# roeiherz/CanonicalSg2Im

Measured on AMD Instinct MI355X. Metric: 256x256 images/sec/node (G+D step), higher is better.
Workload: dtype f32; 1 GPU; BASELINE config C3: COCO-shaped AttSPADE 256x256, batch 16/GPU, 1-30 objects/img, ngf=64 ndf=64, --no_vgg_loss --use_img_disc 0; Sg2Layout GCN + SPADE G + 2-scale PatchGAN D + object-crop D, fwd+bwd+Adam; global_batch=16, parallelism=dp1

## Files before the change

canonicalsg2im_amd/_lib.py:

```python
import ctypes
import os

import torch

_HERE = os.path.dirname(os.path.abspath(__file__))
LIB_PATH = os.environ.get("CSG_HIP_LIB") or os.path.join(_HERE, "libcsg_hip.so")

MAX_TAPS = 16
ACT_NONE, ACT_LEAKY, ACT_TANH = 0, 1, 2

c_i32, c_i64, c_f32, c_f64, c_p = ctypes.c_int32, ctypes.c_int64, ctypes.c_float, ctypes.c_double, ctypes.c_void_p


class ConvDesc(ctypes.Structure):
    _fields_ = [
        ("B", c_i32), ("IHp", c_i32), ("IWp", c_i32), ("Cin", c_i32), ("x_cs", c_i32),
        ("IHv", c_i32), ("IWv", c_i32), ("in_up", c_i32),
        ("OHg", c_i32), ("OWg", c_i32), ("OHf", c_i32), ("OWf", c_i32), ("os", c_i32), ("ooy", c_i32), ("oox", c_i32),
        ("Cout", c_i32), ("y_cs", c_i32),
        ("istride", c_i32), ("ntaps", c_i32), ("wtaps", c_i32),
        ("tap_dy", c_i32 * MAX_TAPS), ("tap_dx", c_i32 * MAX_TAPS), ("tap_w", c_i32 * MAX_TAPS),
        ("act", c_i32), ("slope", c_f32), ("accumulate", c_i32), ("res_gate", c_i32),
    ]

# ... 19 lines not shown

class SnFwdItem(ctypes.Structure):
    _fields_ = [("w", c_p), ("u", c_p), ("v", c_p), ("Cout", c_i64), ("K", c_i64), ("w_eff", c_p), ("cl_Cin", c_i64),
                ("sigma", c_p), ("u_used", c_p), ("v_used", c_p), ("workspace", c_p), ("workspace_bytes", c_i64)]


class SnBwdItem(ctypes.Structure):
    _fields_ = [("dweff", c_p), ("Cout", c_i64), ("Cin", c_i64), ("KH", c_i64), ("KW", c_i64), ("s0", c_i64), ("s1", c_i64),
                ("s2", c_i64), ("s3", c_i64), ("w", c_p), ("u_used", c_p), ("v_used", c_p), ("sigma", c_p), ("dw", c_p),
                ("workspace", c_p), ("workspace_bytes", c_i64)]


class GemmDesc(ctypes.Structure):
    _fields_ = [("M", ctypes.c_int64), ("N", ctypes.c_int64), ("K", ctypes.c_int64),
                ("lda", ctypes.c_int64), ("ldb", ctypes.c_int64), ("ldy", ctypes.c_int64), ("ldg", ctypes.c_int64),
                ("act", ctypes.c_int32), ("slope", ctypes.c_float), ("gate_slope", ctypes.c_float)]


SIGNATURES = {
    "csg_version": (c_i32, []),
    "csg_last_error": (ctypes.c_char_p, []),
    "csg_prof_enable": (c_i32, [c_i32]),
    "csg_prof_reset": (c_i32, []),
    "csg_prof_num_kernels": (c_i32, []),
    "csg_prof_kernel_name": (ctypes.c_char_p, [c_i32]),
    "csg_prof_read": (c_i32, [c_i32, ctypes.POINTER(c_f64), ctypes.POINTER(c_i64), ctypes.POINTER(c_f64)]),
    "csg_embed_fwd": (c_i32, [c_p, c_i64, c_i64, c_p, c_i64, c_i64, c_p, c_i64, c_i64, c_p]),
    "csg_embed_bwd_workspace": (c_i64, [c_i64, c_i64, c_i64]),
    "csg_embed_bwd": (c_i32, [c_p, c_i64, c_i64, c_p, c_i64, c_i64, c_i64, c_i64, c_p, c_p, c_i64, c_p]),
    "csg_real_object_mask": (c_i32, [c_p, c_i64, c_i64, c_i64, c_i64, c_p, c_p]),
    "csg_graph_csr_build": (c_i32, [c_p, c_i64, c_i64, c_i64, c_p, c_p, c_p]),
    "csg_gather_concat_fwd": (c_i32, [c_p, c_p, c_p, c_i64, c_i64, c_i64, c_i64, c_i64, c_p, c_p]),
    "csg_gather_concat_bwd_workspace": (c_i64, [c_i64, c_i64, c_i64, c_i64]),
    "csg_gather_concat_bwd": (c_i32, [c_p, c_p, c_p, c_i64, c_i64, c_i64, c_i64, c_i64, c_p, c_p, c_p, c_i64, c_p]),
    "csg_segment_avg_fwd_workspace": (c_i64, [c_i64, c_i64, c_i64, c_i64]),
    "csg_segment_avg_fwd": (c_i32, [c_p, c_p, c_p, c_p, c_p, c_i64, c_i64, c_i64, c_i64, c_i64, c_p, c_p, c_p, c_p,
                                    c_i64, c_p]),
    "csg_segment_avg_bwd": (c_i32, [c_p, c_p, c_p, c_p, c_p, c_p, c_p, c_p, c_i64, c_i64, c_i64, c_i64, c_i64, c_i32,
                                    c_p, c_p, c_p, c_p]),
    "csg_layout_fwd": (c_i32, [c_p, c_p, c_p, c_p, c_i64, c_i64, c_i64, c_i64, c_i64, c_i64, c_i64, c_i64, c_p, c_i64,
                               c_i64, c_p]),
    "csg_disc_input_fwd": (c_i32, [c_p, c_p, c_p, c_p, c_i64, c_i64, c_i64, c_i64, c_i64, c_i64, c_p, c_i64, c_i64, c_i64,
                                   c_i64, c_p, c_i64, c_p]),
    "csg_layout_bwd_workspace": (c_i64, [c_i64, c_i64, c_i64, c_i64, c_i64, c_i32, c_i32]),
    "csg_layout_bwd": (c_i32, [c_p, c_i64, c_i64, c_p, c_p, c_p, c_i64, c_i64, c_i64, c_i64, c_i64, c_i64, c_i64,
                               c_i64, c_p, c_i32, c_p, c_p, c_p, c_i64, c_p]),
    "csg_layout_bwd_masks": (c_i32, [c_p, c_i64, c_i64, c_p, c_p, c_i64, c_i64, c_i64, c_i64, c_i64, c_i64, c_i64, c_i64,
                                     c_p, c_p, c_i32, c_p]),
    "csg_layout_mass": (c_i32, [c_p, c_p, c_p, c_p, c_i64, c_i64, c_i64, c_i64, c_i64, c_i64, c_p, c_p]),
    "csg_layout_paint": (c_i32, [c_p, c_p, c_p, c_i64, c_p, c_i64, c_i64, c_i64, c_i64, c_i64, c_i64, c_i64, c_p, c_i64,
                                 c_i64, c_p]),
    "csg_conv_fwd_workspace": (c_i64, [ctypes.POINTER(ConvDesc)]),
    "csg_conv_fwd": (c_i32, [ctypes.POINTER(ConvDesc), c_p, c_p, c_p, c_p, c_p, c_p, c_i64, c_p]),
    "csg_conv_bwd_weight_workspace": (c_i64, [ctypes.POINTER(ConvDesc)]),
    "csg_conv_bwd_weight": (c_i32, [ctypes.POINTER(ConvDesc), c_p, c_p, c_p, c_p, c_p, c_i64, c_p]),
    "csg_wino_pack_bytes": (c_i64, [c_i64, c_i64]),
    "csg_wino_pack_weights": (c_i32, [c_p, c_i64, c_i64, c_i64, c_i64, c_i64, c_i64, c_i32, c_p, c_p, c_p]),
    "csg_conv_fwd_multi_workspace": (c_i64, [ctypes.POINTER(ConvDesc), c_i32]),
    "csg_conv_fwd_multi": (c_i32, [ctypes.POINTER(ConvDesc), c_i32, c_p, c_p, c_p, c_p, c_p, c_p, c_i64, c_p]),
    "csg_gemm_supported": (c_i32, [ctypes.POINTER(GemmDesc)]),
    "csg_gemm_nt": (c_i32, [ctypes.POINTER(GemmDesc), c_p, c_p, c_p, c_p, c_p, c_p]),
    "csg_gemm_tn_workspace": (c_i64, [c_i64, c_i64, c_i64]),
    "csg_gemm_tn": (c_i32, [c_i64, c_i64, c_i64, c_p, c_i64, c_p, c_i64, c_p, c_p, c_p, c_i64, c_p]),
    "csg_conv_few_supported": (c_i32, [ctypes.POINTER(FewDesc)]),
    "csg_conv_few_fwd_workspace": (c_i64, [ctypes.POINTER(FewDesc)]),
    "csg_conv_few_fwd": (c_i32, [ctypes.POINTER(FewDesc), c_p, c_p, c_p, c_p, c_p, c_i64, c_p]),
    "csg_conv_few_bwd_data": (c_i32, [ctypes.POINTER(FewDesc), c_p, c_p, c_p, c_p]),
    "csg_conv_few_bwd_weight_workspace": (c_i64, [ctypes.POINTER(FewDesc)]),
    "csg_conv_few_bwd_weight": (c_i32, [ctypes.POINTER(FewDesc), c_p, c_p, c_p, c_p, c_p, c_i64, c_p]),
    "csg_wino_conv_workspace": (c_i64, [ctypes.POINTER(WinoDesc)]),
    "csg_wino_conv": (c_i32, [ctypes.POINTER(WinoDesc), c_p, c_p, c_p, c_p, c_p, c_f32, c_p, c_p, c_i64, c_p]),
    "csg_wino_bwd_weight_workspace": (c_i64, [ctypes.POINTER(WinoDesc)]),
    "csg_wino_bwd_weight": (c_i32, [ctypes.POINTER(WinoDesc), c_p, c_p, c_p, c_p, c_p, c_i64, c_p]),
    "csg_wino4_bwd_weight_workspace": (c_i64, [ctypes.POINTER(WinoDesc)]),
    "csg_wino4_bwd_weight": (c_i32, [ctypes.POINTER(WinoDesc), c_p, c_p, c_p, c_p, c_p, c_i64, c_p]),
    "csg_wino4_supported": (c_i32, [ctypes.POINTER(WinoDesc)]),
    "csg_wino4_persistent": (c_i32, [c_i32]),
    "csg_wino_pack_weights_multi": (c_i32, [ctypes.POINTER(WinoPackItem), c_i32, c_p]),
    "csg_wino4_pack_bytes": (c_i64, [c_i64, c_i64]),
    "csg_wino4_pack_weights": (c_i32, [c_p, c_i64, c_i64, c_i64, c_i64, c_i64, c_i64, c_i32, c_p, c_p, c_p]),
    "csg_wino4_conv_workspace": (c_i64, [ctypes.POINTER(WinoDesc)]),
    "csg_wino4_conv": (c_i32, [ctypes.POINTER(WinoDesc), c_p, c_p, c_p, c_p, c_p, c_f32, c_p, c_p, c_i64, c_p]),
    "csg_wino4_conv_part": (c_i32, [ctypes.POINTER(WinoDesc), c_p, c_p, c_i64, c_i64, c_p, c_p, c_p, c_i64, c_p, c_p, c_f32,
                                    c_p, c_p]),
    "csg_wino4_conv_spade_supported": (c_i32, [ctypes.POINTER(WinoDesc)]),
    "csg_wino4_conv_spade": (c_i32, [ctypes.POINTER(WinoDesc), c_p, c_p, c_p, c_p, c_p, c_i64, c_p, c_p, c_f32, c_p, c_p]),
    "csg_wino34_supported": (c_i32, [ctypes.POINTER(WinoDesc), c_i32]),
    "csg_wino34_pack_weights": (c_i32, [c_p, c_i64, c_i64, c_i64, c_i64, c_i64, c_i64, c_i32, c_p, c_p, c_p]),
    "csg_wino34_conv_workspace": (c_i64, [ctypes.POINTER(WinoDesc), c_i32]),
    "csg_wino34_conv": (c_i32, [ctypes.POINTER(WinoDesc), c_i32, c_p, c_p, c_p, c_p, c_p, c_f32, c_p, c_p, c_i64, c_p]),
    "csg_act_bwd": (c_i32, [c_p, c_p, c_i64, c_i32, c_f32, c_p, c_p]),
    "csg_colsum": (c_i32, [c_p, c_i64, c_i64, c_i64, c_p, c_p, c_i64, c_p]),
    "csg_norm_stats": (c_i32, [c_p, c_i64, c_i64, c_i64, c_p, c_p, c_i64, c_p]),
    "csg_norm_finalize": (c_i32, [c_p, c_i64, c_i64, c_f64, c_f32, c_i32, c_p, c_p, c_p, c_p, c_f32, c_p]),
    "csg_norm_stats_finalize": (c_i32, [c_p, c_i64, c_i64, c_i64, c_p, c_i64, c_f64, c_f32, c_p, c_p, c_p, c_p, c_p, c_p, c_f32,
                                        c_p]),
    "csg_norm_apply_fwd": (c_i32, [c_p, c_p, c_p, c_p, c_f32, c_i64, c_i64, c_i64, c_p, c_p, c_f32, c_p, c_p]),
    "csg_norm_apply_bwd_reduce": (c_i32, [c_p, c_p, c_p, c_p, c_p, c_p, c_f32, c_i64, c_i64, c_i64, c_p, c_p, c_p, c_i64,
                                          c_i64, c_p]),
    "csg_norm_apply_bwd_dx": (c_i32, [c_p, c_p, c_p, c_p, c_p, c_f32, c_p, c_f64, c_i64, c_i64, c_i64, c_p, c_p, c_p, c_f32,
                                      c_p, c_p, c_i64, c_p]),
    "csg_nearest_resize_fwd": (c_i32, [c_p, c_i64, c_i64, c_i64, c_i64, c_i64, c_i64, c_p, c_p]),
    "csg_nearest_resize_bwd": (c_i32, [c_p, c_i64, c_i64, c_i64, c_i64, c_i64, c_i64, c_p, c_p]),
    "csg_upsample2x_fwd": (c_i32, [c_p, c_i64, c_i64, c_i64, c_i64, c_p, c_p]),
    "csg_upsample2x_bwd": (c_i32, [c_p, c_i64, c_i64, c_i64, c_i64, c_p, c_p]),
    "csg_avgpool3s2_fwd": (c_i32, [c_p, c_i64, c_i64, c_i64, c_i64, c_p, c_p]),
    "csg_avgpool3s2_bwd": (c_i32, [c_p, c_i64, c_i64, c_i64, c_i64, c_p, c_p]),
    "csg_avgpool3s2_bwd_add": (c_i32, [c_p, c_i64, c_i64, c_i64, c_i64, c_p, c_p, c_p]),
    "csg_crop_fwd": (c_i32, [c_p, c_i64, c_i64, c_i64, c_i64, c_i64, c_p, c_p, c_i64, c_i64, c_i64, c_p, c_i64, c_p]),
    "csg_crop_bwd": (c_i32, [c_p, c_i64, c_i64, c_i64, c_i64, c_i64, c_p, c_p, c_i64, c_i64, c_i64, c_i64, c_p, c_p]),
    "csg_crop_bwd_boxes": (c_i32, [c_p, c_p, c_i64, c_i64, c_i64, c_i64, c_i64, c_p, c_p, c_i64, c_i64, c_i64, c_i64, c_p,
                                   c_p]),
    "csg_maxpool2_fwd": (c_i32, [c_p, c_i64, c_i64, c_i64, c_i64, c_p, c_p]),
    "csg_maxpool2_bwd": (c_i32, [c_p, c_p, c_i64, c_i64, c_i64, c_i64, c_p, c_p]),
    "csg_avgpool2_fwd": (c_i32, [c_p, c_i64, c_i64, c_i64, c_i64, c_p, c_p]),
    "csg_avgpool2_bwd": (c_i32, [c_p, c_i64, c_i64, c_i64, c_i64, c_p, c_p]),
    "csg_l1_mean_workspace": (c_i64, [c_i64]),
    "csg_l1_mean_fwd": (c_i32, [c_p, c_p, c_i64, c_p, c_p, c_i64, c_p]),
    "csg_l1_mean_bwd": (c_i32, [c_p, c_p, c_p, c_i64, c_p, c_p]),
    "csg_hinge_mean_fwd": (c_i32, [ctypes.POINTER(HingeItem), c_i32, c_i32, c_p, c_p]),
    "csg_hinge_mean_bwd": (c_i32, [ctypes.POINTER(HingeItem), c_i32, c_i32, c_p, c_p]),
    "csg_spectral_norm_workspace": (c_i64, [c_i64, c_i64]),
    "csg_spectral_norm_fwd": (c_i32, [c_p, c_p, c_p, c_i64, c_i64, c_i32, c_f32, c_p, c_i64, c_p, c_p, c_p, c_p, c_i64,
                                      c_p]),
    "csg_spectral_norm_bwd": (c_i32, [c_p, c_i64, c_i64, c_i64, c_i64, c_i64, c_i64, c_i64, c_i64, c_p, c_p, c_p, c_p,
                                      c_p, c_p, c_i64, c_p]),
    "csg_spectral_norm_fwd_multi": (c_i32, [ctypes.POINTER(SnFwdItem), c_i32, c_i32, c_f32, c_p]),
    "csg_spectral_norm_bwd_multi": (c_i32, [ctypes.POINTER(SnBwdItem), c_i32, c_p]),
    "csg_canon_workspace": (c_i64, [c_i64]),
    "csg_canon_build": (c_i32, [c_p, c_p, c_p, c_p, c_i64, c_i64, ctypes.POINTER(c_i32), c_i64, c_i32, c_i32, c_p, c_i64,
                                c_p, c_p]),
    "csg_canon_emit": (c_i32, [c_p, c_p, c_i64, c_i64, ctypes.POINTER(c_i32), c_i64, c_i32, c_i32, c_p, c_p, c_i64, c_p,
                               c_p, c_p]),
    "csg_canon_converse": (c_i32, [c_p, c_p, c_i64, c_i64, ctypes.POINTER(c_i32), c_i64, c_i32, c_i32, c_p, c_p, c_p, c_p,
                                   c_i64, c_p, c_p, c_p]),
    "csg_canon_general_workspace": (c_i64, [c_i64, c_i64, c_i64]),
    "csg_canon_general_build": (c_i32, [c_p, c_p, c_p, c_p, c_i64, c_i64, c_p, c_p, c_i64, ctypes.POINTER(c_i32), c_i64,
                                        c_i64, c_i32, c_p, c_i64, c_p, c_p]),
    "csg_canon_general_converse": (c_i32, [c_i64, ctypes.POINTER(c_i32), c_i64, c_p, c_i64, c_p, c_p, c_p, c_p, c_p]),
    "csg_canon_general_close": (c_i32, [c_i64, ctypes.POINTER(c_i32), c_i64, c_i32, c_p, c_i64, c_p, c_p]),
    "csg_canon_general_emit": (c_i32, [c_i64, ctypes.POINTER(c_i32), c_i64, c_p, c_i64, c_p, c_i64, c_p, c_p, c_p]),
}


def _load():
    if not os.path.exists(LIB_PATH):
        raise ImportError(
            "libcsg_hip.so is not built (%s). Run `python -c 'import __graft_entry__ as g; g.build()'` "
            "from the repository root; there is no CPU fallback." % LIB_PATH)
    lib = ctypes.CDLL(LIB_PATH)
    for name, (res, args) in SIGNATURES.items():
        fn = getattr(lib, name)
        fn.restype = res
        fn.argtypes = args
    return lib


lib = _load()


def last_error():
    return lib.csg_last_error().decode("utf-8", "replace")


def check(rc, what=""):
    if rc != 0:
        raise RuntimeError("libcsg_hip %s failed (%d): %s" % (what, rc, last_error()))


def ptr(t):
    if t is None:
        return None
    if not t.is_cuda:
        raise RuntimeError("canonicalsg2im_amd ops need HIP (cuda) tensors; got a %s tensor — there is no CPU path"
                           % t.device)
    return ctypes.c_void_p(t.data_ptr())


_raw_stream = getattr(torch._C, "_cuda_getCurrentRawStream", None)


def stream():
    if _raw_stream is not None:
        return ctypes.c_void_p(_raw_stream(torch.cuda.current_device()))
    return ctypes.c_void_p(torch.cuda.current_stream().cuda_stream)


def prof_enable(on=True):
    check(lib.csg_prof_enable(int(on)), "prof_enable")


def prof_reset():
    check(lib.csg_prof_reset(), "prof_reset")


def prof_read():
    out = {}
    for k in range(lib.csg_prof_num_kernels()):
        ms, n, w = c_f64(), c_i64(), c_f64()
        check(lib.csg_prof_read(k, ctypes.byref(ms), ctypes.byref(n), ctypes.byref(w)), "prof_read")
        if n.value:
            out[lib.csg_prof_kernel_name(k).decode()] = (ms.value, n.value, w.value)
    return out
```

canonicalsg2im_amd/csrc/igemm.hip:

```cpp
#include <stddef.h>
#include <stdlib.h>

#include <type_traits>

#include "csg_common.h"
#include "csg_reduce.h"

using namespace csg;

typedef __attribute__((ext_vector_type(16))) float f32x16;
typedef float f32x4 __attribute__((ext_vector_type(4)));
typedef int i32x4 __attribute__((ext_vector_type(4)));

__device__ f32x4 csg_buffer_load_f32x4(i32x4 rsrc, int voffset, int soffset, int aux) __asm(
    "llvm.amdgcn.raw.buffer.load.v4f32");

__device__ __forceinline__ i32x4 make_srd(const void* base, unsigned bytes) {
  const unsigned long long a = (unsigned long long)base;
  i32x4 r;
  r.x = (int)(a & 0xffffffffu);
  r.y = (int)((a >> 32) & 0xffffu);
  r.z = (int)bytes;
  r.w = 0x00020000;
  return r;
}

#define IG_BM 128
#define IG_BK 32
#define IG_LD 36
#define OOB_OFF 0x80000000u
#define MAX_RECORDS 0x7FFFFFF0ll

struct FastDiv {
  unsigned m, s1, s2;
};
static FastDiv make_fastdiv(unsigned d) {
  FastDiv f;
  unsigned l = 0;
  while ((1ull << l) < d) ++l;
  f.m = (unsigned)(((1ull << 32) * ((1ull << l) - d)) / d + 1);
  f.s1 = l < 1 ? l : 1;
  f.s2 = l > 0 ? l - 1 : 0;
  return f;
}
__device__ __forceinline__ unsigned fdiv(unsigned n, const FastDiv& f) {
  unsigned t = __umulhi(f.m, n);
  return (t + ((n - t) >> f.s1)) >> f.s2;
}

struct IgemmParams {
  csg_conv_desc d;
  int M, Ktot, wrow;
  int mtiles, ntiles;
  int simple_out;
  int ksplit, kt_per_split;
// ... 557 lines not shown
  }
  const int left = ch1 - ch;
  if (left == 3) {
    load_tile(ch + 2, ra0, rb0);
    compute_store(buf, ra1, rb1);
    __syncthreads();
    compute_store(buf ^ 1, ra0, rb0);
    __syncthreads();
    compute_tile(buf);
  } else if (left == 2) {
    compute_store(buf, ra1, rb1);
    __syncthreads();
    compute_tile(buf ^ 1);
  } else if (left == 1) {
    compute_tile(buf);
  }

  float* slab = out + (long long)sp * d.Cout * p.wrow;
#pragma unroll
  for (int mi = 0; mi < MI; ++mi) {
    const int n = it * BI + wi * (MI * 32) + r * MI + mi;
    if (n >= d.Cout) continue;
    float* srow = slab + (long long)n * p.wrow;
#pragma unroll
    for (int g = 0; g < 4; ++g)
#pragma unroll
      for (int f = 0; f < NJ; ++f) {
        const int kk = jt * 128 + wj * (NJ * 32) + (8 * g + 4 * hh) * NJ + 4 * f;
        if (kk < p.Ktot) {
          const int sl = kk / d.Cin;
          const int col = s_tap[32 + sl] * d.Cin + (kk - sl * d.Cin);
          float v[4];
#pragma unroll
          for (int e = 0; e < 4; ++e) {
            const int L = 4 * f + e;
            v[e] = acc[mi][L % NJ][4 * g + L / NJ];
          }
          *(float4*)(srow + col) = make_float4(v[0], v[1], v[2], v[3]);
        }
      }
  }
  if (do_db) {
    __syncthreads();
    f32x4* red = (f32x4*)smem;
    red[apr * CQ + ac4] = csum;
    __syncthreads();
    if (apr == 0 && n0 < d.Cout) {
      f32x4 tot = red[ac4];
      for (int q = 1; q < RP; ++q) tot += red[q * CQ + ac4];
      *(f32x4*)(dbp + (long long)sp * d.Cout + n0) = tot;
    }
  }
}

static int validate(const csg_conv_desc* d, const char* who) {
  CSG_REQUIRE(d != nullptr, CSG_E_BADSHAPE, "%s: null descriptor", who);
  CSG_REQUIRE(d->B > 0 && d->IHp > 0 && d->IWp > 0 && d->Cin > 0 && d->Cout > 0 && d->OHg > 0 && d->OWg > 0,
              CSG_E_BADSHAPE, "%s: non-positive dimension", who);
  CSG_REQUIRE(d->Cin % 4 == 0 && d->x_cs % 4 == 0 && d->x_cs >= d->Cin, CSG_E_UNSUPPORTED,
              "%s: Cin=%d and x_cs=%d must be multiples of 4 (16-byte channel rows)", who, d->Cin, d->x_cs);
  CSG_REQUIRE(d->ntaps >= 1 && d->ntaps <= CSG_MAX_TAPS && d->wtaps >= 1, CSG_E_UNSUPPORTED, "%s: ntaps=%d", who,
              d->ntaps);
  CSG_REQUIRE(d->in_up >= 0 && d->in_up <= 4 && d->os >= 1 && d->istride >= 1, CSG_E_BADSHAPE, "%s: bad strides", who);
  CSG_REQUIRE(d->y_cs >= d->Cout, CSG_E_BADSHAPE, "%s: y_cs < Cout", who);
  for (int t = 0; t < d->ntaps; ++t)
    CSG_REQUIRE(d->tap_w[t] >= 0 && d->tap_w[t] < d->wtaps, CSG_E_BADSHAPE, "%s: tap_w out of range", who);
  int64_t M = (int64_t)d->B * d->OHg * d->OWg;
  CSG_REQUIRE(M < (1ll << 31) - 256, CSG_E_UNSUPPORTED, "%s: too many output pixels", who);
  CSG_REQUIRE((int64_t)d->B * d->OHf * d->OWf < (1ll << 31), CSG_E_UNSUPPORTED, "%s: output too large", who);
  const int64_t img_bytes = (int64_t)d->IHp * d->IWp * d->x_cs * 4;
  const int64_t npix = (int64_t)d->OHg * d->OWg;
  const int64_t span = (127 / npix + 2) * img_bytes;
  CSG_REQUIRE(span < MAX_RECORDS, CSG_E_UNSUPPORTED, "%s: one input image is too large for 32-bit offsets", who);
  CSG_REQUIRE((int64_t)d->Cout * d->wtaps * d->Cin * 4 < MAX_RECORDS, CSG_E_UNSUPPORTED, "%s: weights too large", who);
  return CSG_OK;
}

static void fill(IgemmParams& p, const csg_conv_desc* d) {
  p.d = *d;
  p.M = d->B * d->OHg * d->OWg;
  p.Ktot = d->ntaps * d->Cin;
  p.wrow = d->wtaps * d->Cin;
  p.simple_out = (d->os == 1 && d->ooy == 0 && d->oox == 0 && d->OHg == d->OHf && d->OWg == d->OWf) ? 1 : 0;
  p.ksplit = 1;
  p.kt_per_split = (p.Ktot + IG_BK - 1) / IG_BK;
  p.div_ow = make_fastdiv((unsigned)d->OWg);
  p.div_oh = make_fastdiv((unsigned)d->OHg);
  p.img_bytes = (unsigned)((int64_t)d->IHp * d->IWp * d->x_cs * 4);
  p.mtiles = p.ntiles = 0;
  p.ws_off = 0;
  p.tail_tile0 = p.tail_ks = p.tail_kt_per = p.tail_m0 = 0;
}

static int pick_bn(int cout) { return cout <= 32 ? 32 : (cout <= 64 ? 64 : 128); }

static int pick_split(int blocks, int steps, int min_steps, int max_split) {
  int best = 1;
  double best_cost = 1e30;
  for (int s = 1; s <= max_split && steps / s >= min_steps; ++s) {
    const double rounds = (double)((blocks * (long long)s + 511) / 512);
    const double cost = rounds * ((steps + s - 1) / s) + 0.25 * s;
    if (cost < best_cost * 0.97) {
      best_cost = cost;
      best = s;
    }
  }
// ... 78 lines not shown
}

static int pick_bi(int cout) { return cout <= 32 ? 32 : (cout <= 64 ? 64 : 128); }

static int multi_plan(const csg_conv_desc* descs, int n, IgemmMulti& mp, int64_t& ws_floats, int& max_blocks,
                      const char* who) {
  CSG_REQUIRE(descs != nullptr && n >= 1 && n <= IG_MAXCLS, CSG_E_BADSHAPE, "%s: 1..%d descriptors", who, IG_MAXCLS);
  int64_t blocks_total = 0;
  for (int c = 0; c < n; ++c) {
    int rc = validate(&descs[c], who);
    if (rc) return rc;
    CSG_REQUIRE(descs[c].Cout == descs[0].Cout && descs[c].Cin == descs[0].Cin && descs[c].x_cs == descs[0].x_cs &&
                    descs[c].y_cs == descs[0].y_cs && descs[c].wtaps == descs[0].wtaps && descs[c].B == descs[0].B,
                CSG_E_BADSHAPE, "%s: the descriptors must share channels, strides, weights and batch", who);
    fill(mp.p[c], &descs[c]);
    const int bn = pick_bn(descs[c].Cout);
    mp.p[c].mtiles = (mp.p[c].M + IG_BM - 1) / IG_BM;
    mp.p[c].ntiles = (descs[c].Cout + bn - 1) / bn;
    blocks_total += (int64_t)mp.p[c].mtiles * mp.p[c].ntiles;
  }
  for (int c = n; c < IG_MAXCLS; ++c) mp.p[c] = mp.p[0];
  ws_floats = 0;
  max_blocks = 0;
  for (int c = 0; c < n; ++c) {
    IgemmParams& p = mp.p[c];
    const int nkt = (p.Ktot + IG_BK - 1) / IG_BK;
    int ks = 1;
    if (blocks_total < 1024 && nkt >= 16 && p.d.Cout % 4 == 0) ks = pick_split((int)blocks_total, nkt, 8, 64);
    p.kt_per_split = (nkt + ks - 1) / ks;
    p.ksplit = (nkt + p.kt_per_split - 1) / p.kt_per_split;
    p.ws_off = ws_floats;
    if (p.ksplit > 1) ws_floats += (int64_t)p.ksplit * p.M * p.d.Cout;
    const int blocks = p.mtiles * p.ntiles * p.ksplit;
    if (blocks > max_blocks) max_blocks = blocks;
  }
  return CSG_OK;
}

template <int BN>
static int launch_fwd_multi(IgemmMulti& mp, int n, int max_blocks, const float* x, const float* w, const float* bias,
                            const float* res, float* y, float* ws, hipStream_t s) {
  static bool attr_set = false;
  size_t shm = (size_t)(2 * IG_BM * IG_LD + 2 * BN * IG_LD) * 4 + 48 * 4;
  if (!attr_set) {
    hipError_t e = hipFuncSetAttribute((const void*)k_igemm_fwd<BN, true>, hipFuncAttributeMaxDynamicSharedMemorySize, (int)shm);
    CSG_REQUIRE(e == hipSuccess, CSG_E_LAUNCH, "csg_conv_fwd_multi: hipFuncSetAttribute(%zu bytes of LDS): %s", shm, hipGetErrorString(e));
    attr_set = true;
  }
  CSG_LAUNCH((k_igemm_fwd<BN, true>), dim3((unsigned)max_blocks, (unsigned)n), dim3(256), shm, s, mp, x, w, bias, res,
                     y, ws);
  return check_launch("csg_conv_fwd_multi");
}

extern "C" {

int64_t csg_conv_fwd_workspace(const csg_conv_desc* d) {
  if (validate(d, "csg_conv_fwd_workspace")) return -1;
  IgemmParams p;
  fill(p, d);
  fwd_plan(p);
  return fwd_slab_floats(p) * 4;
}

int csg_conv_fwd(const csg_conv_desc* d, const float* x, const float* w, const float* bias, const float* residual,
                 float* y, float* workspace, int64_t workspace_bytes, void* stream) {
  int rc = validate(d, "csg_conv_fwd");
  if (rc) return rc;
  CSG_REQUIRE(((uintptr_t)x % 16) == 0 && ((uintptr_t)w % 16) == 0, CSG_E_UNSUPPORTED,
              "csg_conv_fwd: x and w must be 16-byte aligned");
  CSG_REQUIRE(!d->res_gate || (d->act == CSG_ACT_NONE && residual != nullptr && !d->accumulate), CSG_E_UNSUPPORTED,
              "csg_conv_fwd: res_gate needs act == NONE, a residual (the gating tensor) and no accumulation");
  IgemmParams p;
  fill(p, d);
  fwd_plan(p);
  const int64_t need = fwd_slab_floats(p) * 4;
  CSG_REQUIRE(need == 0 || (workspace != nullptr && workspace_bytes >= need), CSG_E_WORKSPACE,
              "csg_conv_fwd: needs %lld bytes of workspace (csg_conv_fwd_workspace), got %lld", (long long)need,
              (long long)workspace_bytes);
  hipStream_t s = (hipStream_t)stream;
  const int bn = pick_bn(d->Cout);
  {
    ProfScope ps(bn == 128 ? K_IGEMM_FWD : K_IGEMM_FWD64, 2.0 * p.M * (double)p.Ktot * d->Cout, s);
    if (bn == 32)
      rc = launch_fwd<32>(p, x, w, bias, residual, y, workspace, s);
    else if (bn == 64)
      rc = launch_fwd<64>(p, x, w, bias, residual, y, workspace, s);
    else
      rc = launch_fwd<128>(p, x, w, bias, residual, y, workspace, s);
    if (rc) return rc;
  }
  if (p.ksplit > 1 || p.tail_ks > 1) {
    ProfScope ps(K_SPLITK_EPI, (double)fwd_slab_floats(p) * 4 + (double)(p.M - p.tail_m0) * d->Cout * 4, s);
    const int64_t n4 = (int64_t)(p.M - p.tail_m0) * d->Cout / 4;
    int64_t g = cdiv(n4, 256);
    if (g > 4096) g = 4096;
    CSG_LAUNCH(k_splitk_epilogue<false>, dim3((unsigned)g), dim3(256), 0, s, p, workspace, bias, residual, y);
    rc = check_launch("csg_conv_fwd(split-K epilogue)");
  }
  return rc;
}

int64_t csg_conv_fwd_multi_workspace(const csg_conv_desc* descs, int32_t n) {
  IgemmMulti mp;
  int64_t wsf = 0;
  int mb = 0;
  if (multi_plan(descs, n, mp, wsf, mb, "csg_conv_fwd_multi_workspace")) return -1;
  return wsf * 4;
}

int csg_conv_fwd_multi(const csg_conv_desc* descs, int32_t n, const float* x, const float* w, const float* bias,
                       const float* residual, float* y, float* workspace, int64_t workspace_bytes, void* stream) {
  IgemmMulti mp;
  int64_t wsf = 0;
  int mb = 0;
  int rc = multi_plan(descs, n, mp, wsf, mb, "csg_conv_fwd_multi");
  if (rc) return rc;
  CSG_REQUIRE(((uintptr_t)x % 16) == 0 && ((uintptr_t)w % 16) == 0, CSG_E_UNSUPPORTED,
              "csg_conv_fwd_multi: x and w must be 16-byte aligned");
  CSG_REQUIRE(wsf == 0 || (workspace != nullptr && workspace_bytes >= wsf * 4), CSG_E_WORKSPACE,
              "csg_conv_fwd_multi: needs %lld bytes of workspace", (long long)(wsf * 4));
  hipStream_t s = (hipStream_t)stream;
  const int bn = pick_bn(descs[0].Cout);
  double flops = 0.0;
  bool any_split = false;
  int64_t max_n4 = 0;
  for (int c = 0; c < n; ++c) {
    flops += 2.0 * mp.p[c].M * (double)mp.p[c].Ktot * descs[c].Cout;
    any_split = any_split || mp.p[c].ksplit > 1;
    const int64_t n4 = (int64_t)mp.p[c].M * descs[c].Cout / 4;
    if (n4 > max_n4) max_n4 = n4;
  }
  {
    ProfScope ps(bn == 128 ? K_IGEMM_FWD : K_IGEMM_FWD64, flops, s);
// ... 80 lines not shown
```

include/csg_hip.h:

```cpp
#ifndef CSG_HIP_H
#define CSG_HIP_H

#include <stdint.h>

#ifdef __cplusplus
extern "C" {
#endif

#define CSG_OK 0
#define CSG_E_BADSHAPE (-1)
#define CSG_E_UNSUPPORTED (-2)
#define CSG_E_LAUNCH (-3)
#define CSG_E_WORKSPACE (-4)

#define CSG_ACT_NONE 0
#define CSG_ACT_LEAKY 1
#define CSG_ACT_TANH 2

#define CSG_MAX_TAPS 16

int csg_version(void);
const char* csg_last_error(void);

int csg_prof_enable(int mode);
// ... 18 lines not shown
int csg_gather_concat_fwd(const float* obj, const float* pred, const int64_t* triplets, int64_t B, int64_t O,
                          int64_t T, int64_t Din, int64_t Dp, float* out, void* stream);
int64_t csg_gather_concat_bwd_workspace(int64_t B, int64_t O, int64_t T, int64_t Din);
int csg_gather_concat_bwd(const float* dcat, const int32_t* row_ptr, const int32_t* col, int64_t B, int64_t O,
                          int64_t T, int64_t Din, int64_t Dp, float* dobj, float* dpred, void* workspace,
                          int64_t workspace_bytes, void* stream);

int64_t csg_segment_avg_fwd_workspace(int64_t B, int64_t O, int64_t T, int64_t H);
int csg_segment_avg_fwd(const float* h, const float* conf, const uint8_t* valid, const int32_t* row_ptr,
                        const int32_t* col, int64_t B, int64_t O, int64_t T, int64_t H, int64_t Dp, float* pooled,
                        float* cnt, float* new_p, void* workspace, int64_t workspace_bytes, void* stream);
int csg_segment_avg_bwd(const float* dpooled, const float* dnew_p, const float* h, const float* conf,
                        const uint8_t* valid, const int64_t* triplets, const float* pooled, const float* cnt,
                        int64_t B, int64_t O, int64_t T, int64_t H, int64_t Dp, int32_t gate_relu, float* dh,
                        float* dconf, float* dcnt_scratch, void* stream);

int csg_layout_fwd(const float* vecs, const float* boxes, const uint8_t* valid, const float* masks, int64_t M,
                   int64_t B, int64_t O, int64_t S, int64_t H, int64_t W, int64_t OH, int64_t OW, float* out,
                   int64_t out_cs, int64_t out_off, void* stream);
int csg_disc_input_fwd(const float* vecs, const float* boxes, const uint8_t* valid, const float* masks, int64_t M, int64_t B,
                       int64_t O, int64_t S, int64_t H, int64_t W, const float* img, int64_t img_sb, int64_t img_sc,
                       int64_t img_sh, int64_t img_sw, float* out, int64_t out_cs, void* stream);
int64_t csg_layout_bwd_workspace(int64_t B, int64_t O, int64_t S, int64_t OH, int64_t OW, int32_t has_masks,
                                 int32_t box_gradients);
int csg_layout_bwd(const float* dout, int64_t out_cs, int64_t out_off, const float* boxes, const uint8_t* valid,
                   const float* masks, int64_t M, int64_t B, int64_t O, int64_t S, int64_t H, int64_t W, int64_t OH,
                   int64_t OW, float* dvecs, int accumulate, const float* vecs, float* dboxes, void* workspace,
                   int64_t workspace_bytes, void* stream);
int csg_layout_bwd_masks(const float* dout, int64_t out_cs, int64_t out_off, const float* boxes, const uint8_t* valid,
                         int64_t M, int64_t B, int64_t O, int64_t S, int64_t H, int64_t W, int64_t OH, int64_t OW,
                         const float* vecs, float* dmasks, int accumulate, void* stream);
int csg_layout_mass(const float* vecs, const float* boxes, const uint8_t* valid, const float* masks, int64_t M,
                    int64_t B, int64_t O, int64_t S, int64_t H, int64_t W, float* mass, void* stream);
int csg_layout_paint(const float* vecs, const float* boxes, const float* masks, int64_t M, const int32_t* order,
                     int64_t B, int64_t O, int64_t S, int64_t H, int64_t W, int64_t OH, int64_t OW, float* out,
                     int64_t out_cs, int64_t out_off, void* stream);

typedef struct csg_conv_desc {
  int32_t B, IHp, IWp, Cin, x_cs;
  int32_t IHv, IWv, in_up;
  int32_t OHg, OWg, OHf, OWf, os, ooy, oox;
  int32_t Cout, y_cs;
  int32_t istride, ntaps, wtaps;
  int32_t tap_dy[CSG_MAX_TAPS], tap_dx[CSG_MAX_TAPS], tap_w[CSG_MAX_TAPS];
  int32_t act;
  float slope;
  int32_t accumulate;
  int32_t res_gate;
} csg_conv_desc;

int64_t csg_conv_fwd_workspace(const csg_conv_desc* d);
int csg_conv_fwd(const csg_conv_desc* d, const float* x, const float* w, const float* bias, const float* residual,
                 float* y, float* workspace, int64_t workspace_bytes, void* stream);
int64_t csg_conv_fwd_multi_workspace(const csg_conv_desc* descs, int32_t n);
int csg_conv_fwd_multi(const csg_conv_desc* descs, int32_t n, const float* x, const float* w, const float* bias,
                       const float* residual, float* y, float* workspace, int64_t workspace_bytes, void* stream);
int64_t csg_conv_bwd_weight_workspace(const csg_conv_desc* d);
int csg_conv_bwd_weight(const csg_conv_desc* d, const float* x, const float* dy, float* dw, float* db,
                        float* workspace, int64_t workspace_bytes, void* stream);

typedef struct csg_wino_desc {
  int32_t B, H, W;
  int32_t Cin, x_cs;
  int32_t Cout, y_cs;
  int32_t act;
  float slope;
} csg_wino_desc;
int64_t csg_wino_pack_bytes(int64_t N, int64_t K);
int csg_wino_pack_weights(const float* w, int64_t s_o, int64_t s_i, int64_t s_h, int64_t s_w, int64_t Cout, int64_t Cin,
                          int32_t backward_data, const float* sigma, float* packed, void* stream);
int64_t csg_wino_conv_workspace(const csg_wino_desc* d);
int csg_wino_conv(const csg_wino_desc* d, const float* x, const float* packed, const float* bias,
                  const float* residual, const float* gate, float gate_slope, float* y, float* workspace,
                  int64_t workspace_bytes, void* stream);
int64_t csg_wino_bwd_weight_workspace(const csg_wino_desc* d);
int csg_wino_bwd_weight(const csg_wino_desc* d, const float* x, const float* dy, float* dw, float* db, float* workspace,
                        int64_t workspace_bytes, void* stream);

int64_t csg_wino4_bwd_weight_workspace(const csg_wino_desc* d);
int csg_wino4_bwd_weight(const csg_wino_desc* d, const float* x, const float* dy, float* dw, float* db, float* workspace,
                         int64_t workspace_bytes, void* stream);

int32_t csg_wino4_supported(const csg_wino_desc* d);
typedef struct csg_wino_pack_item {
  const float* w;
  int64_t s_o, s_i, s_h, s_w;
  int64_t Cout, Cin;
  int32_t backward_data;
  int32_t variant;
  float* packed;
} csg_wino_pack_item;
int csg_wino_pack_weights_multi(const csg_wino_pack_item* items, int32_t n, void* stream);
int32_t csg_wino4_persistent(int32_t on);
int64_t csg_wino4_pack_bytes(int64_t N, int64_t K);
int csg_wino4_pack_weights(const float* w, int64_t s_o, int64_t s_i, int64_t s_h, int64_t s_w, int64_t Cout, int64_t Cin,
                           int32_t backward_data, const float* sigma, float* packed, void* stream);
int64_t csg_wino4_conv_workspace(const csg_wino_desc* d);
int csg_wino4_conv(const csg_wino_desc* d, const float* x, const float* packed, const float* bias,
                   const float* residual, const float* gate, float gate_slope, float* y, float* workspace,
                   int64_t workspace_bytes, void* stream);

int csg_wino4_conv_part(const csg_wino_desc* d, const float* x, const float* packed, int64_t tile_off, int64_t tiles_total,
                        const float* bias, const float* mod_x, const float* mod_gamma, int64_t gamma_cs,
                        const float* mod_mean, const float* mod_invstd, float mod_slope, float* y, void* stream);

int32_t csg_wino4_conv_spade_supported(const csg_wino_desc* d);
// ... 175 lines not shown
```

Before: 217.8 img/s.

## Add dedicated dense-row MFMA kernel for 4x4 stride-2 discriminator convs

Adds a specialized implicit-GEMM forward kernel for 4x4 stride-2, pad-2 convolutions, the PatchGAN discriminator layers. It precomputes per-row tap validity masks, DMAs A/B tiles straight into LDS with buffer_load_lds and double-buffers the stages. A small cost model picks a split-K factor, and the existing split-K epilogue reduces the partial results. It is on by default and can be disabled with an env var. The aim is to beat the generic igemm path's per-tap address handling on these layers, at the cost of extra code paths and workspace-size changes.

```diff
diff --git a/canonicalsg2im_amd/_lib.py b/canonicalsg2im_amd/_lib.py
--- a/canonicalsg2im_amd/_lib.py
+++ b/canonicalsg2im_amd/_lib.py
@@ -95,6 +95,8 @@
                                  c_i64, c_p]),
     "csg_conv_fwd_workspace": (c_i64, [ctypes.POINTER(ConvDesc)]),
     "csg_conv_fwd": (c_i32, [ctypes.POINTER(ConvDesc), c_p, c_p, c_p, c_p, c_p, c_p, c_i64, c_p]),
+    "csg_conv_s2_dense_enable": (c_i32, [c_i32]),
+    "csg_conv_s2_dense_launches": (c_i64, []),
     "csg_conv_bwd_weight_workspace": (c_i64, [ctypes.POINTER(ConvDesc)]),
     "csg_conv_bwd_weight": (c_i32, [ctypes.POINTER(ConvDesc), c_p, c_p, c_p, c_p, c_p, c_i64, c_p]),
     "csg_wino_pack_bytes": (c_i64, [c_i64, c_i64]),
@@ -200,6 +202,8 @@
 
 
 lib = _load()
+if os.environ.get("CSG_CONV_S2_DENSE", "1") == "0":
+    lib.csg_conv_s2_dense_enable(0)
 
 
 def last_error():
diff --git a/canonicalsg2im_amd/csrc/igemm.hip b/canonicalsg2im_amd/csrc/igemm.hip
--- a/canonicalsg2im_amd/csrc/igemm.hip
+++ b/canonicalsg2im_amd/csrc/igemm.hip
@@ -1,6 +1,7 @@
 #include <stddef.h>
 #include <stdlib.h>
 
+#include <atomic>
 #include <type_traits>
 
 #include "csg_common.h"
@@ -664,6 +665,211 @@
     }
   }
 }
+
+struct S2Params {
+  int B, IH, IW, Cin, x_cs, OH, OW, Cout, y_cs, act;
+  float slope;
+  int M, K, nnb, nstage, ksplit, st_per;
+  FastDiv div_ow, div_oh;
+  unsigned img_bytes;
+};
+
+typedef __attribute__((address_space(3))) void* ig_lds_ptr;
+
+template <int NTW, int BK>
+__global__ __launch_bounds__(256, BK == 16 ? 4 : 2) void k_conv_s2_fwd(S2Params p, const float* __restrict__ x,
+                                                                       const float* __restrict__ w,
+                                                                       const float* __restrict__ bias,
+                                                                       float* __restrict__ y, float* __restrict__ ws) {
+  constexpr int BN = 64 * NTW;
+  constexpr int SLOTS = BK / 4;
+  constexpr int SH = BK == 32 ? 1 : 2;
+  constexpr int NA = 128 * SLOTS / 256, NB = BN * SLOTS / 256;
+  constexpr int RPI = 256 / SLOTS;
+  constexpr int ASZ = 128 * BK, STG = (128 + BN) * BK;
+  constexpr int G = BK / 8;
+  extern __shared__ __attribute__((aligned(16))) float smem[];
+  const int tid = threadIdx.x, lane = tid & 63, wave = tid >> 6;
+  const int c = lane & 31, h = lane >> 5;
+  const int wm = wave & 1, wn = wave >> 1;
+  int bid = xcd_remap(blockIdx.x, gridDim.x);
+  const int ks = bid % p.ksplit;
+  bid /= p.ksplit;
+  const int nb = bid % p.nnb, mb = bid / p.nnb;
+  const int m0 = mb * 128, n0 = nb * BN;
+  const int mrem = p.M - m0, nrem = p.Cout - n0;
+  const int s_begin = ks * p.st_per, s_end = min(p.nstage, s_begin + p.st_per);
+
+  const int b0 = (int)fdiv(fdiv((unsigned)m0, p.div_ow), p.div_oh);
+  const long long a_rem = (long long)(p.B - b0) * p.img_bytes;
+  const __amdgpu_buffer_rsrc_t rsA = __builtin_amdgcn_make_buffer_rsrc(
+      (void*)(x + (long long)b0 * (p.img_bytes >> 2)), 0, (int)(a_rem < MAX_RECORDS ? a_rem : MAX_RECORDS), 0x00020000);
+  const float* Bb = w + (long long)n0 * p.K;
+  const __amdgpu_buffer_rsrc_t rsB = __builtin_amdgcn_make_buffer_rsrc(
+      (void*)Bb, 0, (int)((long long)min(nrem, BN) * p.K * 4), 0x00020000);
+
+  const int row0 = tid / SLOTS;
+  const int kslot = (tid & (SLOTS - 1)) ^ ((row0 >> SH) & (SLOTS - 1));
+  int offA[NA];
+  unsigned maskA[NA];
+  unsigned offB[NB];
+#pragma unroll
+  for (int i = 0; i < NA; ++i) {
+    const int m = m0 + row0 + RPI * i;
+    const bool ok = m < p.M;
+    const unsigned t = fdiv((unsigned)(ok ? m : 0), p.div_ow);
+    const int ox = (int)((unsigned)(ok ? m : 0) - t * (unsigned)p.OW);
+    const unsigned bb = fdiv(t, p.div_oh);
+    const int oy = (int)(t - bb * (unsigned)p.OH);
+    const int iy0 = 2 * oy - 2, ix0 = 2 * ox - 2;
+    offA[i] = (int)(((unsigned)((int)bb - b0)) * p.img_bytes) + (iy0 * p.IW + ix0) * p.x_cs * 4;
+    unsigned ym = 0, xm = 0;
+#pragma unroll
+    for (int k = 0; k < 4; ++k) {
+      ym |= ((unsigned)(iy0 + k) < (unsigned)p.IH ? 1u : 0u) << (4 * k);
+      xm |= ((unsigned)(ix0 + k) < (unsigned)p.IW ? 1u : 0u) << k;
+    }
+    maskA[i] = ok ? ym * xm : 0u;
+  }
+#pragma unroll
+  for (int i = 0; i < NB; ++i) offB[i] = (unsigned)((row0 + RPI * i) * p.K + kslot * 4) * 4u;
+  int tap, cch;
+  {
+    const int k = s_begin * BK + kslot * 4;
+    tap = k / p.Cin;
+    cch = k - tap * p.Cin;
+  }
+  auto dma_stage = [&](int s, int bufsel) {
+    const bool kin = s < s_end;
+    float* base = smem + bufsel * STG + wave * 256;
+    const int tapoff = (((tap >> 2) * p.IW + (tap & 3)) * p.x_cs + cch) * 4;
+    const unsigned tbit = kin ? (1u << tap) : 0u;
+#pragma unroll
+    for (int i = 0; i < NA; ++i)
+      __builtin_amdgcn_raw_ptr_buffer_load_lds(rsA, (ig_lds_ptr)(base + i * 1024), 16,
+                                               (int)((maskA[i] & tbit) ? (unsigned)(offA[i] + tapoff) : OOB_OFF), 0, 0, 0);
+#pragma unroll
+    for (int i = 0; i < NB; ++i)
+      __builtin_amdgcn_raw_ptr_buffer_load_lds(rsB, (ig_lds_ptr)(base + ASZ + i * 1024), 16,
+                                               (int)(kin ? offB[i] : OOB_OFF), s * BK * 4, 0, 0);
+    cch += BK;
+    const bool wrap = cch >= p.Cin;
+    cch = wrap ? cch - p.Cin : cch;
+    tap = wrap ? tap + 1 : tap;
+  };
+
+  const int sw = (c >> SH) & (SLOTS - 1);
+  int ra[G], rb[G];
+#pragma unroll
+  for (int g = 0; g < G; ++g) {
+    const int slot = ((2 * g + h) ^ sw) * 4;
+    ra[g] = (wm * 64 + c) * BK + slot;
+    rb[g] = ASZ + (wn * 32 * NTW + c) * BK + slot;
+  }
+  struct Frag {
+    f32x4 a[2], b[NTW];
+  };
+  auto read_frag = [&](int bufsel, int g, Frag& f) {
+    const float* s = smem + bufsel * STG;
+    f.a[0] = *(const f32x4*)(s + ra[g]);
+    f.a[1] = *(const f32x4*)(s + ra[g] + 32 * BK);
+#pragma unroll
+    for (int nt = 0; nt < NTW; ++nt) f.b[nt] = *(const f32x4*)(s + rb[g] + nt * 32 * BK);
+  };
+
+  f32x16 acc[2][NTW];
+#pragma unroll
+  for (int mt = 0; mt < 2; ++mt)
+#pragma unroll
+    for (int nt = 0; nt < NTW; ++nt)
+#pragma unroll
+      for (int e = 0; e < 16; ++e) acc[mt][nt][e] = 0.f;
+
+  auto compute = [&](const Frag& f) {
+#pragma unroll
+    for (int j = 0; j < 4; ++j) {
+#pragma unroll
+      for (int mt = 0; mt < 2; ++mt)
+#pragma unroll
+        for (int nt = 0; nt < NTW; ++nt)
+          acc[mt][nt] = __builtin_amdgcn_mfma_f32_32x32x2f32(f.b[nt][j], f.a[mt][j], acc[mt][nt], 0, 0, 0);
+    }
+  };
+
+  auto stage_barrier = [&]() {
+    __builtin_amdgcn_s_waitcnt(0x0F70);
+    __builtin_amdgcn_s_barrier();
+  };
+  Frag f[2];
+  dma_stage(s_begin, 0);
+  stage_barrier();
+  __builtin_amdgcn_sched_barrier(0);
+  read_frag(0, 0, f[0]);
+  int buf = 0;
+  for (int s = s_begin; s < s_end; ++s) {
+    dma_stage(s + 1, buf ^ 1);
+    __builtin_amdgcn_sched_barrier(0);
+#pragma unroll
+    for (int g = 0; g + 1 < G; ++g) {
+      read_frag(buf, g + 1, f[(g + 1) & 1]);
+      __builtin_amdgcn_sched_barrier(0);
+      compute(f[g & 1]);
+      __builtin_amdgcn_sched_barrier(0);
+    }
+    stage_barrier();
+    __builtin_amdgcn_sched_barrier(0);
+    if (s + 1 < s_end) read_frag(buf ^ 1, 0, f[0]);
+    compute(f[(G - 1) & 1]);
+    __builtin_amdgcn_sched_barrier(0);
+    buf ^= 1;
+  }
+
+  int ncol[NTW][4];
+  bool nin[NTW][4];
+  f32x4 bv[NTW][4];
+  const bool raw = p.ksplit > 1;
+#pragma unroll
+  for (int nt = 0; nt < NTW; ++nt)
+#pragma unroll
+    for (int q = 0; q < 4; ++q) {
+      ncol[nt][q] = wn * 32 * NTW + nt * 32 + 8 * q + 4 * h;
+      nin[nt][q] = ncol[nt][q] < nrem;
+      bv[nt][q] = f32x4{0.f, 0.f, 0.f, 0.f};
+      if (!raw && bias != nullptr && nin[nt][q]) bv[nt][q] = *(const f32x4*)(bias + n0 + ncol[nt][q]);
+    }
+  __builtin_amdgcn_sched_barrier(0);
+  if (!raw) {
+#pragma unroll
+    for (int mt = 0; mt < 2; ++mt)
+#pragma unroll
+      for (int nt = 0; nt < NTW; ++nt)
+#pragma unroll
+        for (int q = 0; q < 4; ++q)
+#pragma unroll
+          for (int u = 0; u < 4; ++u) {
+            float v = acc[mt][nt][4 * q + u] + bv[nt][q][u];
+            if (p.act == CSG_ACT_LEAKY) v = v > 0.f ? v : v * p.slope;
+            acc[mt][nt][4 * q + u] = v;
+          }
+  }
+  __builtin_amdgcn_sched_barrier(0);
+  float* obase = raw ? ws + (long long)ks * p.M * p.Cout : y;
+  const int ld = raw ? p.Cout : p.y_cs;
+#pragma unroll
+  for (int mt = 0; mt < 2; ++mt) {
+    const int m = wm * 64 + mt * 32 + c;
+    const bool mok = m < mrem;
+    float* yrow = obase + (long long)(m0 + m) * ld + n0;
+#pragma unroll
+    for (int nt = 0; nt < NTW; ++nt)
+#pragma unroll
+      for (int q = 0; q < 4; ++q)
+        if (mok && nin[nt][q])
+          *(f32x4*)(yrow + ncol[nt][q]) =
+              f32x4{acc[mt][nt][4 * q], acc[mt][nt][4 * q + 1], acc[mt][nt][4 * q + 2], acc[mt][nt][4 * q + 3]};
+  }
+}
+
 
 static int validate(const csg_conv_desc* d, const char* who) {
   CSG_REQUIRE(d != nullptr, CSG_E_BADSHAPE, "%s: null descriptor", who);
@@ -848,6 +1054,61 @@
   return check_launch("csg_conv_fwd_multi");
 }
 
+static std::atomic<int> g_s2_on{1};
+static std::atomic<long long> g_s2_launches{0};
+
+static bool s2_desc_ok(const csg_conv_desc* d) {
+  if (!g_s2_on.load(std::memory_order_relaxed)) return false;
+  if (d->ntaps != 16 || d->wtaps != 16 || d->istride != 2 || d->in_up != 0 || d->os != 1 || d->ooy != 0 || d->oox != 0)
+    return false;
+  if (d->OHg != d->OHf || d->OWg != d->OWf || d->IHv != d->IHp || d->IWv != d->IWp) return false;
+  if (d->OHg != d->IHp / 2 + 1 || d->OWg != d->IWp / 2 + 1) return false;
+  if (d->Cin < 32 || d->Cin % 4 || d->x_cs % 4 || d->Cout % 4 || d->y_cs % 4) return false;
+  if (d->accumulate || d->res_gate || (d->act != CSG_ACT_NONE && d->act != CSG_ACT_LEAKY)) return false;
+  for (int t = 0; t < 16; ++t)
+    if (d->tap_dy[t] != t / 4 - 2 || d->tap_dx[t] != t % 4 - 2 || d->tap_w[t] != t) return false;
+  return true;
+}
+
+static void s2_plan(const csg_conv_desc* d, S2Params& p, int& ntw) {
+  ntw = d->Cout <= 64 ? 1 : 2;
+  const int bk = ntw == 1 ? 32 : 16;
+  p.B = d->B, p.IH = d->IHp, p.IW = d->IWp, p.Cin = d->Cin, p.x_cs = d->x_cs, p.OH = d->OHg, p.OW = d->OWg;
+  p.Cout = d->Cout, p.y_cs = d->y_cs, p.act = d->act, p.slope = d->slope;
+  p.M = d->B * d->OHg * d->OWg;
+  p.K = 16 * d->Cin;
+  p.nnb = (d->Cout + 64 * ntw - 1) / (64 * ntw);
+  p.nstage = p.K / bk;
+  p.div_ow = make_fastdiv((unsigned)d->OWg);
+  p.div_oh = make_fastdiv((unsigned)d->OHg);
+  p.img_bytes = (unsigned)((int64_t)d->IHp * d->IWp * d->x_cs * 4);
+  const int64_t blocks = (int64_t)((p.M + 127) / 128) * p.nnb;
+  const double t_stage = 0.85, slab_us = (double)p.M * d->Cout * 8.0 / 3.5e6;
+  int best = 1;
+  double best_cost = 1e30;
+  for (int ks = 1; ks <= 16 && p.nstage / ks >= 8; ++ks) {
+    const double load = (double)((blocks * ks + 255) / 256);
+    const double cost = load * ((p.nstage + ks - 1) / ks) * t_stage + (ks > 1 ? ks * slab_us + 6.0 : 0.0);
+    if (cost < best_cost * 0.97) {
+      best_cost = cost;
+      best = ks;
+    }
+  }
+  p.st_per = (p.nstage + best - 1) / best;
+  p.ksplit = (p.nstage + p.st_per - 1) / p.st_per;
+}
+
+static int64_t s2_slab_floats(const S2Params& p) { return p.ksplit > 1 ? (int64_t)p.ksplit * p.M * p.Cout : 0; }
+
+template <int NTW, int BK>
+static int launch_s2(const S2Params& p, const float* x, const float* w, const float* bias, float* y, float* ws,
+                     hipStream_t s) {
+  const size_t shm = (size_t)2 * (128 + 64 * NTW) * BK * 4;
+  const unsigned grid = (unsigned)((int64_t)((p.M + 127) / 128) * p.nnb * p.ksplit);
+  CSG_LAUNCH((k_conv_s2_fwd<NTW, BK>), dim3(grid), dim3(256), shm, s, p, x, w, bias, y, ws);
+  return check_launch("csg_conv_fwd(dense-row 4x4/2)");
+}
+
 extern "C" {
 
 int64_t csg_conv_fwd_workspace(const csg_conv_desc* d) {
@@ -855,8 +1116,22 @@
   IgemmParams p;
   fill(p, d);
   fwd_plan(p);
-  return fwd_slab_floats(p) * 4;
-}
+  int64_t need = fwd_slab_floats(p);
+  if (s2_desc_ok(d)) {
+    S2Params sp;
+    int ntw;
+    s2_plan(d, sp, ntw);
+    if (s2_slab_floats(sp) > need) need = s2_slab_floats(sp);
+  }
+  return need * 4;
+}
+
+int csg_conv_s2_dense_enable(int on) {
+  g_s2_on.store(on != 0 ? 1 : 0);
+  return CSG_OK;
+}
+
+int64_t csg_conv_s2_dense_launches(void) { return (int64_t)g_s2_launches.load(); }
 
 int csg_conv_fwd(const csg_conv_desc* d, const float* x, const float* w, const float* bias, const float* residual,
                  float* y, float* workspace, int64_t workspace_bytes, void* stream) {
@@ -868,13 +1143,37 @@
               "csg_conv_fwd: res_gate needs act == NONE, a residual (the gating tensor) and no accumulation");
   IgemmParams p;
   fill(p, d);
+  hipStream_t s = (hipStream_t)stream;
+  const int bn = pick_bn(d->Cout);
+  if (residual == nullptr && s2_desc_ok(d) && ((uintptr_t)y % 16) == 0 && ((uintptr_t)bias % 16) == 0) {
+    S2Params sp;
+    int ntw;
+    s2_plan(d, sp, ntw);
+    const int64_t need = s2_slab_floats(sp) * 4;
+    CSG_REQUIRE(need == 0 || (workspace != nullptr && workspace_bytes >= need), CSG_E_WORKSPACE,
+                "csg_conv_fwd: needs %lld bytes of workspace (csg_conv_fwd_workspace), got %lld", (long long)need,
+                (long long)workspace_bytes);
+    {
+      ProfScope ps(bn == 128 ? K_IGEMM_FWD : K_IGEMM_FWD64, 2.0 * p.M * (double)p.Ktot * d->Cout, s);
+      rc = ntw == 1 ? launch_s2<1, 32>(sp, x, w, bias, y, workspace, s) : launch_s2<2, 16>(sp, x, w, bias, y, workspace, s);
+      if (rc) return rc;
+    }
+    g_s2_launches.fetch_add(1);
+    if (sp.ksplit > 1) {
+      p.ksplit = sp.ksplit;
+      ProfScope ps(K_SPLITK_EPI, (double)s2_slab_floats(sp) * 4 + (double)p.M * d->Cout * 4, s);
+      int64_t g = cdiv((int64_t)p.M * d->Cout / 4, 256);
+      if (g > 4096) g = 4096;
+      CSG_LAUNCH(k_splitk_epilogue<false>, dim3((unsigned)g), dim3(256), 0, s, p, workspace, bias, residual, y);
+      rc = check_launch("csg_conv_fwd(split-K epilogue)");
+    }
+    return rc;
+  }
   fwd_plan(p);
   const int64_t need = fwd_slab_floats(p) * 4;
   CSG_REQUIRE(need == 0 || (workspace != nullptr && workspace_bytes >= need), CSG_E_WORKSPACE,
               "csg_conv_fwd: needs %lld bytes of workspace (csg_conv_fwd_workspace), got %lld", (long long)need,
               (long long)workspace_bytes);
-  hipStream_t s = (hipStream_t)stream;
-  const int bn = pick_bn(d->Cout);
   {
     ProfScope ps(bn == 128 ? K_IGEMM_FWD : K_IGEMM_FWD64, 2.0 * p.M * (double)p.Ktot * d->Cout, s);
     if (bn == 32)
diff --git a/include/csg_hip.h b/include/csg_hip.h
--- a/include/csg_hip.h
+++ b/include/csg_hip.h
@@ -94,6 +94,8 @@
 int64_t csg_conv_fwd_workspace(const csg_conv_desc* d);
 int csg_conv_fwd(const csg_conv_desc* d, const float* x, const float* w, const float* bias, const float* residual,
                  float* y, float* workspace, int64_t workspace_bytes, void* stream);
+int csg_conv_s2_dense_enable(int on);
+int64_t csg_conv_s2_dense_launches(void);
 int64_t csg_conv_fwd_multi_workspace(const csg_conv_desc* descs, int32_t n);
 int csg_conv_fwd_multi(const csg_conv_desc* descs, int32_t n, const float* x, const float* w, const float* bias,
                        const float* residual, float* y, float* workspace, int64_t workspace_bytes, void* stream);
```

After: 217.6 img/s. Within noise of the previous version (-0.1%).
